# alexisvannson/GraphNet_Classifier

Hardware: AMD Instinct MI355X
Metric: edges aggregated/sec (GraphNet forward) (higher is better)
Workload: dtype f32; 1 GPU; c3: 1M nodes / 10M edges (6250 graphs x 160 nodes x 1600 edges), D=64, 2 GN blocks; graphs=6250, nodes=1000000, edges=10000000, n_blocks=2, width=64, step=CSR build + GraphNet.forward, inputs resident in HBM

## Files before the change

### graphnet_classifier_amd/GNN.py

```python
from __future__ import annotations

import os

import torch
import torch.nn as nn
from torch import Tensor

from . import functional as Fn
from . import native
from .MLP import MLP, default_device, require_gpu_param
from .topology import GraphTopology, get_destination_csr, get_topology


WSPLIT = os.environ.get("GNC_NO_WSPLIT") is None
READOUT_HIP = os.environ.get("GNC_NO_READOUT_KERNEL") is None
FUSED_AGG = os.environ.get("GNC_NO_FUSED_AGG") is None


def scatter_sum(src: Tensor, index: Tensor, dim: int = 0, dim_size: int | None = None) -> Tensor:
    if dim != 0:
        raise NotImplementedError("fallback scatter_sum currently supports dim=0 only")
    if src.ndim == 1:
        src = src.unsqueeze(-1)
    if dim_size is None:
        dim_size = int(index.max().item()) + 1 if index.numel() > 0 else 0
    dev = src.device if src.is_cuda else default_device()
    if dev.type != "cuda":
        raise RuntimeError("scatter_sum: no GPU visible and no CPU fallback exists")
    out_device = src.device
    csr = get_destination_csr(index, dim_size, dev)
    src = src.to(device=dev, dtype=torch.float32)
# ... 11 lines not shown

class EdgeProcessor(nn.Module):
    def __init__(self, in_dim_node: int, in_dim_edge: int, hidden_dim: int = 128, hidden_layers: int = 2,
                 activation: str = "ReLU", initializer: None | str = None, norm_type: None | str = "LayerNorm"):
        super().__init__()
        self.edge_processor = MLP(2 * in_dim_node + in_dim_edge, in_dim_edge, hidden_dim, hidden_layers, activation,
                                  initializer, norm_type)

    def forward(self, src, dest, edge_attr, u=None, batch=None):
        dev = require_gpu_param(self.edge_processor.model[0].weight, "EdgeProcessor")
        back = edge_attr.device
        src, dest, edge_attr = (t.to(device=dev, dtype=torch.float32) for t in (src, dest, edge_attr))
        out = self.edge_processor.forward_segments([(src, None), (dest, None), (edge_attr, None)], residual=edge_attr)
        return out if back == dev else out.to(back)

    def forward_sorted(self, x: Tensor, topo: GraphTopology, edge_attr: Tensor, aggregate: bool = False):
        mlp = self.edge_processor
        norm = mlp.model[-1] if mlp.norm_type is not None else None
        lin = mlp._linears()
        trainable_split = mlp.activation_name == "ReLU" or not torch.is_grad_enabled()
        if (WSPLIT and trainable_split and not isinstance(norm, nn.BatchNorm1d) and mlp.activation_name in native.ACTIVATIONS
                and lin[0].in_features == 2 * x.size(1) + edge_attr.size(1) and x.size(1) % 4 == 0):
            ln = (norm.weight, norm.bias, norm.eps) if isinstance(norm, nn.LayerNorm) else None
            if aggregate and not torch.is_grad_enabled():
                return Fn.edge_processor_wsplit_aggregated(x, edge_attr, topo, [m.weight for m in lin], [m.bias for m in lin],
                                                           ln, mlp.activation_name, mlp._act_param())
            if aggregate:
                return Fn.edge_processor_wsplit(x, edge_attr, topo, [m.weight for m in lin], [m.bias for m in lin], ln,
                                                mlp.activation_name, mlp._act_param(), with_agg=True)
            return Fn.edge_processor_wsplit(x, edge_attr, topo, [m.weight for m in lin],
                                            [m.bias for m in lin], ln, mlp.activation_name, mlp._act_param())
        out = mlp.forward_segments(
            [(x, topo.src_sorted), (x, topo.dst_sorted), (edge_attr, None)], residual=edge_attr, rows=topo.num_edges)
        return (out, None) if aggregate else out


class NodeProcessor(nn.Module):
    def __init__(self, in_dim_node: int, in_dim_edge: int, hidden_dim: int = 128, hidden_layers: int = 2,
                 activation: str = "ReLU", initializer: None | str = None, norm_type: None | str = "LayerNorm"):
        super().__init__()
        self.node_processor = MLP(in_dim_node + in_dim_edge, in_dim_node, hidden_dim, hidden_layers, activation,
# ... 26 lines not shown

    def forward(self, x: Tensor, edge_index: Tensor, edge_attr: Tensor | None = None, u=None, batch=None):
        dev = require_gpu_param(next(self.parameters()), "MetaLayer")
        back = x.device
        x = x.to(device=dev, dtype=torch.float32)
        edge_attr = edge_attr.to(device=dev, dtype=torch.float32)
        topo = get_topology(edge_index, x.size(0), dev)
        e_sorted = Fn.permute_rows(edge_attr, topo.perm, topo.inv_perm)
        x, e_sorted = self.forward_sorted(x, topo, e_sorted)
        edge_attr = Fn.permute_rows(e_sorted, topo.inv_perm, topo.perm)
        x, edge_attr = _poison_if_deferred(topo, x), _poison_if_deferred(topo, edge_attr)
        if back != dev:
            x, edge_attr = x.to(back), edge_attr.to(back)
        return x, edge_attr, u

    def forward_sorted(self, x: Tensor, topo: GraphTopology, edge_attr: Tensor):
        agg = None
        if self.edge_model is not None:
            if (FUSED_AGG and self.node_model is not None
                    and isinstance(self.edge_model, EdgeProcessor) and isinstance(self.node_model, NodeProcessor)):
                edge_attr, agg = self.edge_model.forward_sorted(x, topo, edge_attr, aggregate=True)
            else:
                edge_attr = self.edge_model.forward_sorted(x, topo, edge_attr)
        if self.node_model is not None:
            if agg is not None:
                x = self.node_model.forward_sorted(x, topo, edge_attr, agg)
            else:
                x = self.node_model.forward_sorted(x, topo, edge_attr)
        return x, edge_attr


def build_GN_block(in_dim_node: int, in_dim_edge: int, hidden_dim_node: int = 128, hidden_dim_edge: int = 128,
                   hidden_layers_node: int = 2, hidden_layers_edge: int = 2, activation: str = "ReLU",
                   initializer: None | str = None, norm_type: None | str = "LayerNorm"):
    return MetaLayer(
        edge_model=EdgeProcessor(in_dim_node, in_dim_edge, hidden_dim_edge, hidden_layers_edge, activation,
# ... 17 lines not shown
    def forward(self, x, edge_index, edge_attr):
        if len(self.blocks) == 0:
            return x, edge_attr
        dev = require_gpu_param(next(self.parameters()), "GraphProcessor")
        back = x.device
        x = x.to(device=dev, dtype=torch.float32)
        edge_attr = edge_attr.to(device=dev, dtype=torch.float32)
        topo = get_topology(edge_index, x.size(0), dev)
        x, e_sorted = self.forward_sorted(x, topo, Fn.permute_rows(edge_attr, topo.perm, topo.inv_perm))
        edge_attr = Fn.permute_rows(e_sorted, topo.inv_perm, topo.perm)
        x, edge_attr = _poison_if_deferred(topo, x), _poison_if_deferred(topo, edge_attr)
        if back != dev:
            x, edge_attr = x.to(back), edge_attr.to(back)
        return x, edge_attr

    def forward_sorted(self, x, topo: GraphTopology, edge_attr):
        for block in self.blocks:
            x, edge_attr = block.forward_sorted(x, topo, edge_attr)
        return x, edge_attr


class GraphNet(nn.Module):
    def __init__(self, **kwargs):
        super().__init__()
        num_global_features = kwargs.get("num_global_features", 0)
        num_local_features = kwargs.get("num_local_features", 3)
        space_dim = kwargs.get("space_dim", 2)
        in_dim_node = num_local_features + num_global_features
        in_dim_edge = 1 + space_dim
        out_dim = kwargs.get("out_channels", 1)
        n_blocks = kwargs.get("n_blocks", 10)
        out_dim_node = kwargs.get("out_dim_node", 128)
        out_dim_edge = kwargs.get("out_dim_edge", 128)
# ... 19 lines not shown
                                initializer=initializer, norm_type=norm_type)
        self.edge_encoder = MLP(in_dim_edge, out_dim_edge, hidden_dim_edge, hidden_layers_edge, activation=activation,
                                initializer=initializer, norm_type=norm_type)
        self.graph_processor = GraphProcessor(n_blocks, out_dim_node, out_dim_edge, hidden_dim_processor_node,
                                              hidden_dim_processor_edge, hidden_layers_processor_node,
                                              hidden_layers_processor_edge, activation=activation,
                                              initializer=initializer, norm_type=norm_type)
        self.node_decoder = MLP(out_dim_node, out_dim, hidden_dim_decoder, hidden_layers_decoder, norm_type=None)

    def forward_device(self, x: Tensor, pos: Tensor, topo: GraphTopology) -> Tensor:
        out = self.node_encoder.forward_segments([(x.view(x.size(0), -1), None)])
        edge_attr = self.edge_encoder.forward_edge_features(pos, topo.src_sorted, topo.dst_sorted)
        if edge_attr is None:
            edge_attr = Fn.edge_features(pos, topo.src_sorted, topo.dst_sorted)
            edge_attr = self.edge_encoder.forward_segments([(edge_attr, None)])
        out, _ = self.graph_processor.forward_sorted(out, topo, edge_attr)
        out = self.node_decoder.forward_segments([(out, None)])
        return _poison_if_deferred(topo, out)

    def forward(self, x, pos, edge_index):
        dev = require_gpu_param(self.node_encoder.model[0].weight, "GraphNet")
        back = x.device
        x = x.to(device=dev, dtype=torch.float32)
        pos = pos.to(device=dev, dtype=torch.float32)
        topo = get_topology(edge_index, x.size(0), dev)
        out = self.forward_device(x, pos, topo)
        return out if back == dev else out.to(back)


class CapturedForward:

# ... 142 lines not shown
```

### graphnet_classifier_amd/csrc/mlp_device.h

```cpp
#pragma once
#include "gnc_common.h"

namespace gnc_mlp {

typedef float f32x16 __attribute__((ext_vector_type(16)));
typedef float f32x4 __attribute__((ext_vector_type(4)));

constexpr int KC = 64;
constexpr int LDSW = 68;
constexpr int RPW = 32;

__device__ __forceinline__ f32x16 mfma(float a, float b, f32x16 c) {
  return __builtin_amdgcn_mfma_f32_32x32x2f32(a, b, c, 0, 0, 0);
}

__device__ __forceinline__ void wave_lds_fence() {
  asm volatile("s_waitcnt lgkmcnt(0)" ::: "memory");
}

__device__ __forceinline__ float activate(float x, int act, float p) {
  switch (act) {
    case GNC_ACT_RELU: return x < 0.f ? 0.f : x;
    case GNC_ACT_IDENTITY: return x;
    case GNC_ACT_TANH: return tanhf(x);
// ... 745 lines not shown
  float* g_sum;
  int ld_g_sum;
};

__host__ __device__ inline int ldw_of(const gnc_mlp_desc_t& d, int l) { return d.ld_weight[l] ? d.ld_weight[l] : d.in_dim[l]; }

inline int tiles_for(int width) {
  const int t = (width + 31) / 32;
  return t <= 1 ? 1 : t <= 2 ? 2 : t <= 4 ? 4 : 8;
}

int validate_desc(const gnc_mlp_desc_t* d, bool check_ptrs);
int launch_resident_dual(const float* x, int64_t ld_x, int64_t rows, const float* wa, int64_t ld_wa, const float* wb, int64_t ld_wb,
                         int in_dim, int out_dim, float* out_a, float* out_b, int64_t ld_out, hipStream_t stream, bool* launched);
int launch_resident(const gnc_mlp_desc_t& d, int T, bool narrow_out, hipStream_t stream, bool* launched,
                    bool probe_only = false);
int launch_stream(const gnc_mlp_desc_t& d, int T, bool narrow_out, hipStream_t stream, bool* launched,
                  bool probe_only = false);
int launch_stream16(const gnc_mlp_desc_t& d, hipStream_t stream, bool* launched, bool probe_only = false);
int launch_col16(const gnc_mlp_desc_t& d, hipStream_t stream, bool* launched, bool probe_only = false);
int64_t col16_max_rows();
int64_t bwd_col16_max_rows();
bool bwd_col16_supported(const gnc_mlp_desc_t& d);
int bwd_col16_ln_partial_rows(int64_t rows);
int launch_bwd_col16(const gnc_mlp_bwd_desc_t& bd, hipStream_t stream);
bool bwd_col16_persist_supported(const gnc_mlp_desc_t& d);
int bwd_col16_persist_ln_partial_rows(int64_t rows);
int launch_bwd_col16_persist(const gnc_mlp_bwd_desc_t& bd, hipStream_t stream);
bool bwd_stream16_supported(const gnc_mlp_desc_t& d, bool want_dx);
int bwd_stream16_ln_partial_rows(int64_t rows);
int launch_bwd_stream16(const gnc_mlp_desc_t& d, const BwdArgs& b, hipStream_t stream, bool saved = false);
// ... 3 lines not shown
```

### graphnet_classifier_amd/csrc/mlp_fused.hip

```cpp
#include <stdlib.h>

#include "mlp_device.h"

using namespace gnc_mlp;

namespace {

constexpr int WAVES = 4;
constexpr int NT = WAVES * 64;
constexpr int RPB = RPW * WAVES;

__device__ __forceinline__ void stage_rows(float* abuf, const gnc_mlp_segment_t& seg, int64_t row0, int64_t rows,
                                           int c0, int ncol4, bool vec_ok, int lane) {
  const int c4 = lane & 15;
  const int rs = lane >> 4;
  if (c4 < ncol4) {
#pragma unroll
    for (int p = 0; p < RPW / 4; ++p) {
      const int j = p * 4 + rs;
      const int64_t r = row0 + j;
      f32x4 v = {0.f, 0.f, 0.f, 0.f};
      if (r < rows) {
        const int64_t tr = seg.index ? (int64_t)seg.index[r] : r;
        if (!seg.index || (uint64_t)tr < (uint64_t)seg.table_rows)
// ... 232 lines not shown
    rc = launch_stream(probe, T, narrow_out, nullptr, &ok, true);
    if (rc) return rc;
  }
  if (!ok && T == 8) {
    rc = launch_stream16(probe, nullptr, &ok, true);
    if (rc) return rc;
  }
  if (!ok) {
    gnc::set_error("gnc_mlp_agg_supported: needs the weights-resident W-split shape (1 MATMUL + 2 ADD segments, residual = "
                   "the MATMUL segment, widths 33..64) or a 65..128-wide description of the streaming kernel");
    return GNC_ERR_UNSUPPORTED;
  }
  return GNC_OK;
}

namespace {
bool small16(const gnc_mlp_desc_t& d, int T) {
  static const bool off = getenv("GNC_NO_SMALL16") != nullptr;
  return !off && T == 4 && d.rows <= (int64_t)2 * 16 * gnc::num_cu();
}
}

extern "C" int gnc_mlp_save_act_supported(const gnc_mlp_desc_t* desc) {
  int rc = validate_desc(desc, false);
  if (rc) return rc;
  const int L = desc->num_linear;
  int T = tiles_for(desc->out_dim[0]);
  const int od = desc->out_dim[L - 1];
  const bool narrow_out = od <= 32;
  if (!narrow_out && tiles_for(od) > T) T = tiles_for(od);
// ... 167 lines not shown
```

### graphnet_classifier_amd/csrc/mlp_resident.hip

```cpp
#include <stdlib.h>

#include "mlp_device.h"

using namespace gnc_mlp;

#ifdef GNC_PHASE_PROBE
__device__ unsigned long long gnc_phase_probe[4096 * 12];
extern "C" int gnc_phase_probe_read(void* dst, size_t bytes) {
  return (int)hipMemcpyFromSymbol(dst, HIP_SYMBOL(gnc_phase_probe), bytes);
}
#define PROBE_BEGIN() unsigned long long pr_acc[8] = {0, 0, 0, 0, 0, 0, 0, 0}, pr_tp, pr_tn; \
  const unsigned long long pr_c0 = __builtin_readcyclecounter(), pr_w0 = wall_clock64()
#define PROBE_TILE() pr_tp = __builtin_readcyclecounter()
#define PROBE(k) do { pr_tn = __builtin_readcyclecounter(); pr_acc[k] += pr_tn - pr_tp; pr_tp = pr_tn; } while (0)
#define PROBE_END() do { if ((threadIdx.x & 63) == 0) {                                                      \
    unsigned long long* o = gnc_phase_probe + (blockIdx.x * (blockDim.x >> 6) + (threadIdx.x >> 6)) * 12;    \
    for (int k = 0; k < 8; ++k) o[k] = pr_acc[k];                                                            \
    o[8] = __builtin_readcyclecounter() - pr_c0; o[9] = wall_clock64() - pr_w0; } } while (0)
#else
#define PROBE_BEGIN() do {} while (0)
#define PROBE_TILE() do {} while (0)
#define PROBE(k) do {} while (0)
#define PROBE_END() do {} while (0)
#endif

namespace {

constexpr int RWAVES = 8;
constexpr int RNT = RWAVES * 64;

template <int HT, int OT, int NMM, int NADD, bool RESREG, bool AGG = false, bool SAVE = false, bool FULL = false, int EF = 0, bool DUAL = false,
          int SPLIT = 0>
__global__ __launch_bounds__(RNT) void mlp_resident_kernel(const gnc_mlp_desc_t d, const int num_wtiles,
                                                           const int total_chunks) {
  extern __shared__ __attribute__((aligned(16))) float lds[];
  constexpr int WT = HT > OT ? HT : OT;
  constexpr int CH = WT * 32 * LDSW;
  static_assert(SPLIT == 0 || (WT == 2 && NMM == 1 && !DUAL && (SPLIT == 1 || NADD == 0)), "split shapes");
  constexpr int nf32 = SPLIT == 1 ? 0 : NMM;
  __bf16* const wsp = reinterpret_cast<__bf16*>(lds + nf32 * CH);
  auto wsplit = [&](int chunk) -> const __bf16* { return wsp + (chunk - nf32) * 3 * SPLANE; };
  constexpr int PSTRIDE = WT * 32;
  constexpr int NS = NMM + NADD;
  const int tid = threadIdx.x;
  const int lane = tid & 63;
  const int wave = __builtin_amdgcn_readfirstlane(tid >> 6);
  const int i = lane & 31;
// ... 156 lines not shown
  const int col_out = c4 * 4;
  const bool vec_out = FULL || ((out_dim % 4 == 0) && (d.ld_out % 4 == 0) && ((reinterpret_cast<uintptr_t>(d.out) & 15u) == 0));
  const uint32_t out_lane_off = (uint32_t)(rs * d.ld_out + col_out) * 4u;
  const uint32_t res_lane_off = (uint32_t)(rs * d.ld_residual + (col_out < d.ld_residual ? col_out : 0)) * 4u;

  auto agg_ids = [&](int t) -> int {
    int r = t * RPW + (lane & 31);
    r = r < rows ? r : rows - 1;
    return d.agg_index[r];
  };
  int aid = 0, aid_next = 0;
  float agg_acc = 0.f;
  int agg_cur = -1, agg_first_dst = -1;
  bool agg_first = true;
  if constexpr (AGG) aid = agg_ids(wt < last_wt ? wt : last_wt);

  PROBE_BEGIN();
  while (wt < wt_end) {
    PROBE_TILE();
    const int row0 = wt * RPW;
    const int nwt = wt + stride;
    if constexpr (AGG) aid_next = agg_ids(nwt < last_wt ? nwt : last_wt);

    f32x16 hid[HT];
    f32x16 res[RESREG ? HT : 1];
    init_bias<HT>(hid, pbuf, h);
#pragma unroll
    for (int s = 0; s < NMM; ++s) {
      bool interleaved = false;
      if constexpr (EF == 1) ef_stage();
// ... 140 lines not shown
      if constexpr (RESREG) {
#pragma unroll
        for (int t = 0; t < OT && t < HT; ++t) o[t] += res[t < HT ? t : 0];
      }
      compiler_lds_barrier();
      tiles_to_lds<OT>(o, abuf, i, h);
      PROBE(5);
    }
    compiler_lds_barrier();
    if constexpr (AGG) {
      const int valid = rows - row0 < RPW ? rows - row0 : RPW;
      int prv = __shfl_up(aid, 1, 64);
      prv = lane == 0 ? agg_cur : prv;
      const unsigned long long vmask = valid >= 32 ? 0xffffffffull : ((1ull << valid) - 1ull);
      const unsigned long long bnd = __ballot(aid != prv) & vmask;
      float rowv[RPW];
#pragma unroll
      for (int r = 0; r < RPW; ++r) rowv[r] = abuf[r * LDSW + lane];
      auto agg_row = [&](int r) {
        if ((bnd >> r) & 1ull) {
          if (agg_cur >= 0) {
            if (agg_first) {
              agg_first = false;
              agg_first_dst = agg_cur;
            } else if (lane < out_dim) {
              float* dstp = d.agg_out + (int64_t)agg_cur * d.ld_agg;
              asm volatile("s_nop 4\n\tglobal_store_dword %0, %1, %2\n\ts_nop 0" ::"v"(lane * 4), "v"(agg_acc), "s"(dstp) : "memory");
            }
          }
          agg_cur = __builtin_amdgcn_readlane(aid, r);
// ... 17 lines not shown
      aid = aid_next;
    }
    if constexpr (EF == 1) {
      asm volatile("" ::"v"(ef_ps), "v"(ef_pd), "v"(ef_s), "v"(ef_d));
    } else if constexpr (EF == 2) {
      asm volatile("" ::"v"(n3_row.x), "v"(n3_row.y), "v"(n3_row.z));
    } else {
#pragma unroll
      for (int p = 0; p < NP; ++p) asm volatile("" ::"v"(cur[p]));
    }
#pragma unroll
    for (int s = 1; s < NS; ++s) asm volatile("" ::"v"(offs[s]));
    asm volatile("" ::"v"(off0));
    if constexpr (AGG) asm volatile("" ::"v"(aid_next));

    {
      f32x4 outv[NP];
#pragma unroll
      for (int p = 0; p < NP; ++p) outv[p] = *reinterpret_cast<const f32x4*>(abuf + (p * 4 + rs) * LDSW + col_out);
      if (!RESREG && d.residual) {
        f32x4 rv[NP];
        load_tile_rows(rv, d.residual, d.ld_residual, row0, rows, res_lane_off);
#pragma unroll
        for (int p = 0; p < NP; ++p) outv[p] += rv[p];
      }
      if (vec_out) {
        if (col_out < out_dim) {
          if (row0 + RPW <= rows) {
            uint32_t r0b;
            const __amdgpu_buffer_rsrc_t ow = full_tile_window(d.out, row0, rows, d.ld_out, &r0b);
#pragma unroll
// ... 33 lines not shown
    }
    compiler_lds_barrier();
    PROBE(6);
    wt = nwt;
  }
  if constexpr (AGG) {
    if (lane == 0) {
      d.agg_fix[2 * gwave] = agg_first ? agg_cur : agg_first_dst;
      d.agg_fix[2 * gwave + 1] = agg_cur;
    }
  }
  PROBE_END();
}

template <int HT, int OT, int NMM, int NADD, bool RESREG, bool AGG = false, bool SAVE = false, bool FULL = false, int EF = 0, bool DUAL = false,
          int SPLIT = 0>
int launch(const gnc_mlp_desc_t& d, int total_chunks, size_t smem, hipStream_t stream) {
  void (*const kernel)(const gnc_mlp_desc_t, const int, const int) = &mlp_resident_kernel<HT, OT, NMM, NADD, RESREG, AGG, SAVE, FULL, EF, DUAL, SPLIT>;
  static bool attr_set = false;
  if (!attr_set) {
    int rc = gnc::check_hip(hipFuncSetAttribute(reinterpret_cast<const void*>(kernel), hipFuncAttributeMaxDynamicSharedMemorySize, 160 * 1024),
                            "hipFuncSetAttribute(MaxDynamicSharedMemorySize)");
    if (rc) return rc;
    attr_set = true;
  }
  const int64_t num_wtiles = gnc::ceil_div(d.rows, RPW);
  int64_t grid = gnc::ceil_div(num_wtiles, RWAVES);
  if (grid > gnc::num_cu()) grid = gnc::num_cu();
  if constexpr (AGG) grid = gnc::num_cu();
  kernel<<<dim3((unsigned)grid), dim3(RNT), smem, stream>>>(d, (int)num_wtiles, total_chunks);
  return gnc::check_launch("mlp_resident_kernel");
}

template <int HT, int OT, int NMM, int NADD, bool RESREG, bool AGG = false, bool SAVE = false, bool FULL = false, int EF = 0>
int launch_cls(int split, const gnc_mlp_desc_t& d, int total_chunks, size_t smem, hipStream_t stream) {
  if constexpr (HT == 2 && OT == 2 && NMM == 1 && NADD == 2 && RESREG) {
    if (split == 1) return launch<HT, OT, NMM, NADD, RESREG, AGG, SAVE, FULL, EF, false, 1>(d, total_chunks, smem, stream);
  }
  if constexpr (HT == 2 && OT == 2 && NMM == 1 && NADD == 0 && !RESREG && !AGG && !FULL) {
    if (split == 2) return launch<HT, OT, NMM, NADD, RESREG, AGG, SAVE, FULL, EF, false, 2>(d, total_chunks, smem, stream);
  }
  if (split) return GNC_ERR_UNSUPPORTED;
  return launch<HT, OT, NMM, NADD, RESREG, AGG, SAVE, FULL, EF>(d, total_chunks, smem, stream);
}

bool al16(const void* p) { return (reinterpret_cast<uintptr_t>(p) & 15u) == 0; }

}

extern "C" int gnc_mlp_agg_fix_len(void) { return 2 * gnc::num_cu() * RWAVES; }

int gnc_mlp::launch_resident_dual(const float* x, int64_t ld_x, int64_t rows, const float* wa, int64_t ld_wa, const float* wb,
                                  int64_t ld_wb, int in_dim, int out_dim, float* out_a, float* out_b, int64_t ld_out,
                                  hipStream_t stream, bool* launched) {
  *launched = false;
  static const bool disabled = getenv("GNC_MLP_NO_RESIDENT") != nullptr;
  if (disabled || rows < 1 || rows >= INT32_MAX || in_dim < 1 || in_dim > KC || out_dim <= 32 || out_dim > KC || out_dim % 4 != 0 ||
      ld_x % 4 != 0 || ld_x < in_dim || ld_out % 4 != 0 || ld_out < out_dim || ld_wa < in_dim || ld_wb < in_dim || ld_wa > INT32_MAX ||
// ... 13 lines not shown
  d.ld_weight[1] = (int32_t)ld_wb;
  d.in_dim[0] = in_dim;
  d.out_dim[0] = out_dim;
  d.in_dim[1] = in_dim;
  d.out = out_a;
  d.save_act[0] = out_b;
  d.ld_out = (int32_t)ld_out;
  d.rows = rows;
  const int total_chunks = 2;
  const size_t floats = (size_t)total_chunks * 2 * 32 * LDSW + (size_t)(1 + 2) * 2 * 32 + (size_t)RWAVES * RPW * LDSW;
  *launched = true;
  return launch<2, 2, 1, 0, false, false, false, false, 0, true>(d, total_chunks, floats * sizeof(float), stream);
}

int gnc_mlp::launch_resident(const gnc_mlp_desc_t& d, int T, bool narrow_out, hipStream_t stream, bool* launched,
                             bool probe_only) {
  *launched = false;
  static const bool disabled = getenv("GNC_MLP_NO_RESIDENT") != nullptr;
  if (disabled) return GNC_OK;
  if (T > 2 || d.rows >= INT32_MAX) return GNC_OK;
  const int L = d.num_linear;
  const int od = d.out_dim[L - 1];
  if (L > 1 && d.activation != GNC_ACT_RELU) return GNC_OK;
  int nmm = 0, nadd = 0;
  bool n3 = false;
  for (int s = 0; s < d.num_segments; ++s) {
    const gnc_mlp_segment_t& g = d.seg[s];
    if (d.ef_pos && s == 0) continue;
    if (s == 0 && d.num_segments == 1 && !g.index && g.mode == GNC_SEG_MATMUL && g.width == 3 && g.ld == 3 &&
        (reinterpret_cast<uintptr_t>(g.ptr) & 3u) == 0 && d.rows * 12 <= 0xffffffffll && !d.residual && !d.save_act[0] && !d.agg_out &&
        !narrow_out && L >= 2 && T == 2) {
      n3 = true;
// ... 66 lines not shown
    if (d.agg_out && !(nadd == 2 && resreg && d.agg_index && d.agg_fix && d.ld_agg >= od)) return GNC_OK;
    if (nadd == 2 && !resreg) return GNC_OK;
    *launched = true;
    if (probe_only) return GNC_OK;
    if (nmm == 2)
      return resreg ? launch<2, 2, 2, 0, true, false, true>(d, total_chunks, smem, stream)
                    : launch<2, 2, 2, 0, false, false, true>(d, total_chunks, smem, stream);
    if (d.agg_out) return full64 ? launch_cls<2, 2, 1, 2, true, true, true, true>(split, d, total_chunks, smem, stream)
                                 : launch_cls<2, 2, 1, 2, true, true, true>(split, d, total_chunks, smem, stream);
    if (nadd == 2) return launch_cls<2, 2, 1, 2, true, false, true>(split, d, total_chunks, smem, stream);
    return resreg ? launch<2, 2, 1, 0, true, false, true>(d, total_chunks, smem, stream)
                  : launch_cls<2, 2, 1, 0, false, false, true>(split, d, total_chunks, smem, stream);
  }
  if (d.agg_out) {
    if (!(nadd == 2 && nmm == 1 && resreg && !narrow_out && d.agg_index && d.agg_fix && d.ld_agg >= od)) return GNC_OK;
    *launched = true;
    if (probe_only) return GNC_OK;
    if (T == 2 && full64) return launch_cls<2, 2, 1, 2, true, true, false, true>(split, d, total_chunks, smem, stream);
    return T == 2 ? launch_cls<2, 2, 1, 2, true, true>(split, d, total_chunks, smem, stream)
                  : launch<1, 1, 1, 2, true, true>(d, total_chunks, smem, stream);
  }
  if (probe_only) {
    *launched = true;
    return GNC_OK;
  }
#define GNC_RES(HT_, NMM_, NADD_)                                                             \
  do {                                                                                        \
    *launched = true;                                                                         \
    return resreg ? launch<HT_, HT_, NMM_, NADD_, true>(d, total_chunks, smem, stream)        \
                  : launch<HT_, HT_, NMM_, NADD_, false>(d, total_chunks, smem, stream);      \
  } while (0)
  if (narrow_out) {
// ... 20 lines not shown
```

### graphnet_classifier_amd/functional.py

```python
from __future__ import annotations

import torch
import torch.nn.functional as F

import os

from . import native

HIP_BACKWARD = os.environ.get("GNC_TORCH_BACKWARD") is None


def _node_projections(x, w0, dn):
    return native.dual_projection(x, w0[:, :dn], w0[:, dn:2 * dn])


class _ScatterSumCSR(torch.autograd.Function):
    @staticmethod
    def forward(ctx, src, rowptr, perm, dst_of_row, num_nodes):
        ctx.save_for_backward(dst_of_row)
        return native.scatter_sum_csr(src, rowptr, perm, num_nodes)

    @staticmethod
    def backward(ctx, grad_out):
        (dst_of_row,) = ctx.saved_tensors
# ... 385 lines not shown
            dbeta, dgamma = sums[0][:od], sums[0][od:]
        else:
            dbeta, dgamma = r["ln_sums"] if r["ln_sums"] is not None else native.colsum_pair(grad_out, r["yhat"])
        grads[2 + 2 * num_linear] = dgamma
        grads[2 + 2 * num_linear + 1] = dbeta
    return tuple(g if n else None for g, n in zip(grads, need))


def edge_processor_wsplit(x, e, topo, weights, biases, ln, activation="ReLU", act_param=0.0, with_agg=False):
    meta = (topo.src_sorted, topo.dst_sorted, len(weights), activation, float(act_param),
            float(ln[2]) if ln is not None else 0.0, ln is not None, bool(with_agg), torch.is_grad_enabled())
    args = list(weights) + list(biases) + ([ln[0], ln[1]] if ln is not None else [])
    return _EdgeProcessorWSplit.apply(meta, topo, x, e, *args)


def edge_processor_wsplit_aggregated(x, e, topo, weights, biases, ln, activation="ReLU", act_param=0.0):
    dn = x.size(1)
    w0 = weights[0]
    ps, pd = _node_projections(x, w0, dn)
    return native.mlp_forward([(ps, topo.src_sorted), (pd, topo.dst_sorted), (e, None)], [w0[:, 2 * dn:]] + list(weights[1:]),
                              list(biases), ln=ln, activation=activation, act_param=act_param, residual=e, rows=e.size(0),
                              modes=[native.SEG_ADD, native.SEG_ADD, native.SEG_MATMUL],
                              aggregate=(topo.dst_sorted, topo.rowptr, topo.num_nodes))


class _Readout(torch.autograd.Function):

    @staticmethod
    def forward(ctx, y, w1, b1, w2, b2, w3, b3):
        logits, h1, h2 = native.readout_forward(y, w1, b1, w2, b2, w3, b3)
        ctx.save_for_backward(y, w1, w2, w3, h1, h2)
        ctx.has_bias = (b1 is not None, b2 is not None, b3 is not None)
        return logits

    @staticmethod
    def backward(ctx, grad_logits):
        y, w1, w2, w3, h1, h2 = ctx.saved_tensors
        need = ctx.needs_input_grad
# ... 16 lines not shown
```

### graphnet_classifier_amd/native.py

```python
from __future__ import annotations

import ctypes
import os
from ctypes import POINTER, Structure, c_char_p, c_double, c_float, c_int32, c_int64, c_size_t, c_void_p

import torch

LIB_NAME = "libgnc_hip.so"
LIB_PATH = os.path.join(os.path.dirname(os.path.abspath(__file__)), LIB_NAME)

GNC_MAX_SEGMENTS = 4
GNC_MAX_LINEAR = 8
ABI_VERSION = 20

ACTIVATIONS = {
    "ReLU": 0, "Identity": 1, "Tanh": 2, "Sigmoid": 3, "SiLU": 4, "GELU": 5, "LeakyReLU": 6, "ELU": 7,
}

_SIGNATURES = {
    "gnc_abi_version": (c_int32, []),
    "gnc_last_error_string": (c_char_p, []),
    "gnc_target_arch": (c_char_p, []),
    "gnc_mlp_agg_supported": (c_int32, [c_void_p]),
    "gnc_mlp_edge_features_supported": (c_int32, [c_void_p]),
    "gnc_mlp_operands_in_place_supported": (c_int32, [c_void_p]),
    "gnc_mlp_save_act_supported": (c_int32, [c_void_p]),
    "gnc_mlp_agg_fix_len": (c_int32, []),
    "gnc_mlp_small_batch_supported": (c_int32, [c_void_p]),
    "gnc_mlp_small_batch_max_rows": (c_int64, []),
    "gnc_mlp_projection_t2_f32": (c_int32, [c_void_p, c_int64, c_void_p, c_int64, c_int64, c_void_p, c_int64, c_int32, c_int32, c_void_p,
                                            c_int64, c_void_p]),
    "gnc_mlp_dual_projection_f32": (c_int32, [c_void_p, c_int64, c_int64, c_void_p, c_int64, c_void_p, c_int64, c_int32, c_int32,
                                              c_void_p, c_void_p, c_int64, c_void_p]),
    "gnc_mlp_backward_small_batch_supported": (c_int32, [c_void_p]),
    "gnc_readout_forward_f32": (c_int32, [c_void_p, c_int64, c_void_p, c_int64, c_void_p, c_int32, c_void_p, c_int64, c_void_p, c_int32,
                                          c_void_p, c_int64, c_void_p, c_int32, c_void_p, c_void_p, c_void_p, c_void_p, c_void_p]),
    "gnc_readout_backward_f32": (c_int32, [c_void_p, c_void_p, c_int64, c_void_p, c_int64, c_int32, c_void_p, c_int64, c_int32, c_void_p,
                                           c_int64, c_int32, c_void_p, c_void_p, c_void_p, c_void_p, c_void_p, c_void_p, c_void_p, c_void_p,
# ... 446 lines not shown

def _backward_reads_saved_act(lib, desc, any_tensor, need_dx: bool = True) -> bool:
    bd = MlpBwdDesc()
    ctypes.memmove(ctypes.byref(bd.fwd), ctypes.byref(desc), ctypes.sizeof(MlpDesc))
    ptr = any_tensor.data_ptr()
    for l in range(desc.num_linear - 1):
        bd.act[l] = ptr
    bd.act_given, bd.dx = 1, (ptr if need_dx else None)
    if lib.gnc_mlp_backward_fused_rows(ctypes.byref(bd.fwd)) > 0:
        bd.dw_partial[0] = ptr
    return lib.gnc_mlp_backward_saved_act_honoured(ctypes.byref(bd)) == 1


def mlp_forward(segments, weights, biases, ln=None, activation: str = "ReLU", act_param: float = 0.0,
                residual: torch.Tensor | None = None, rows: int | None = None, modes=None, aggregate=None,
                save_act: list | None = None, save_need_dx: bool = True):
    lib = load_library()
    given = (segments, weights, biases, residual, rows, modes)
    small = _rows_of(segments, rows) <= _small_batch_rows(lib)
    raw = not small and save_act is None and aggregate is None
    segs, weights, biases, residual, rows, modes = _prepare_mlp(*given, vector_rows=not (small or raw))
    dev = segs[0][0].device
    out = torch.empty(rows, weights[-1].size(0), dtype=torch.float32, device=dev)
    desc = make_mlp_desc(segs, weights, biases, ln, activation, act_param, residual, out, rows)
    if raw and any(t.data_ptr() % 16 or _ld(t) % 4 for t in [sg[0] for sg in segs] + weights) and \
            lib.gnc_mlp_operands_in_place_supported(ctypes.byref(desc)) != 0:
        segs, weights, biases, residual, rows, modes = _prepare_mlp(*given)
        desc = make_mlp_desc(segs, weights, biases, ln, activation, act_param, residual, out, rows)
    if small and lib.gnc_mlp_small_batch_supported(ctypes.byref(desc)) != 0:
        segs, weights, biases, residual, rows, modes = _prepare_mlp(*given)
        desc = make_mlp_desc(segs, weights, biases, ln, activation, act_param, residual, out, rows)
    if (save_act is not None and SAVE_ACT and rows > 0 and len(weights) >= 2
            and lib.gnc_mlp_save_act_supported(ctypes.byref(desc)) == 0 and _backward_reads_saved_act(lib, desc, out, save_need_dx)):
        for l in range(len(weights) - 1):
            a = torch.empty(rows, weights[l].size(0), dtype=torch.float32, device=dev)
            desc.save_act[l] = a.data_ptr()
            save_act.append(a)
    agg = fix = None
    if aggregate is not None:
        dst_of_row, rowptr, num_nodes = aggregate
        _require_cuda(dst_of_row, rowptr)
        if rows > 0 and lib.gnc_mlp_agg_supported(ctypes.byref(desc)) == 0:
            agg = torch.empty(num_nodes, out.size(1), dtype=torch.float32, device=dev)
            fix = torch.empty(lib.gnc_mlp_agg_fix_len(), dtype=torch.int32, device=dev)
            desc.agg_out, desc.ld_agg = agg.data_ptr(), _ld(agg)
            desc.agg_index, desc.agg_fix = dst_of_row.contiguous().data_ptr(), fix.data_ptr()
    flops = 2.0 * rows * sum(w.size(0) * w.size(1) for w in weights)
    with torch.cuda.device(dev):
        nadd = sum(1 for m in modes if m == SEG_ADD)
        _check(_launch(f"mlp_fused_in{weights[0].size(1)}{'+%dadd' % nadd if nadd else ''}_h{weights[0].size(0)}"
                       f"_out{weights[-1].size(0)}_L{len(weights)}", out,
                       lambda: lib.gnc_mlp_forward_f32(ctypes.byref(desc), _stream(out)), flops),
               "gnc_mlp_forward_f32")
        if agg is not None:
            _check(lib.gnc_agg_fixup_f32(out.data_ptr(), _ld(out), rowptr.data_ptr(), fix.data_ptr(), fix.numel(), num_nodes,
                                         out.size(1), agg.data_ptr(), _ld(agg), _stream(out)), "gnc_agg_fixup_f32")
    return (out, agg) if aggregate is not None else out


FOLD_EDGE_FEATURES = os.environ.get("GNC_NO_K6_FOLD") is None


def mlp_forward_edge_features(pos: torch.Tensor, src: torch.Tensor, dst: torch.Tensor, weights, biases, ln=None,
                              activation: str = "ReLU", act_param: float = 0.0):
    lib = load_library()
    if not FOLD_EDGE_FEATURES or pos.dim() != 2 or pos.size(1) != 2 or src.numel() == 0:
        return None
    _require_cuda(pos, src, dst)
    if src.dtype != torch.int32 or dst.dtype != torch.int32:
        raise TypeError("edge endpoint ids must be int32")
    pos = pos.float().contiguous()
    src, dst = src.contiguous(), dst.contiguous()
# ... 420 lines not shown
```

### include/gnc_hip.h

```cpp
#ifndef GNC_HIP_H
#define GNC_HIP_H

#include <stddef.h>
#include <stdint.h>

#ifdef __cplusplus
extern "C" {
#endif

#define GNC_ABI_VERSION 20

enum {
  GNC_OK = 0,
  GNC_ERR_INVALID_ARGUMENT = -1,
  GNC_ERR_UNSUPPORTED = -2,
  GNC_ERR_WORKSPACE = -3,
  GNC_ERR_HIP = -4
};

#define GNC_MAX_SEGMENTS 4
#define GNC_MAX_LINEAR 8

enum { GNC_ACT_RELU = 0, GNC_ACT_IDENTITY = 1, GNC_ACT_TANH = 2, GNC_ACT_SIGMOID = 3,
       GNC_ACT_SILU = 4, GNC_ACT_GELU = 5, GNC_ACT_LEAKY_RELU = 6, GNC_ACT_ELU = 7 };
// ... 67 lines not shown
  const int32_t* agg_index;
  int32_t* agg_fix;
  float* save_act[GNC_MAX_LINEAR];
  const float* ef_pos;
  const int32_t* ef_src;
  const int32_t* ef_dst;
  int64_t ef_nodes;
  int32_t ef_space_dim;
} gnc_mlp_desc_t;

size_t gnc_sizeof_mlp_desc(void);
int gnc_mlp_supported(const gnc_mlp_desc_t* desc );
int gnc_mlp_forward_f32(const gnc_mlp_desc_t* desc , void* stream);
int gnc_mlp_agg_supported(const gnc_mlp_desc_t* desc );
int gnc_mlp_agg_fix_len(void);
int gnc_mlp_operands_in_place_supported(const gnc_mlp_desc_t* desc );
int gnc_mlp_edge_features_supported(const gnc_mlp_desc_t* desc );
int gnc_mlp_small_batch_supported(const gnc_mlp_desc_t* desc );
int gnc_mlp_projection_t2_f32(const float* a, int64_t ld_a, const float* b, int64_t ld_b, int64_t rows, const float* w, int64_t ld_w,
                              int32_t hidden, int32_t dn, float* out, int64_t ld_out, void* stream);
int64_t gnc_mlp_small_batch_max_rows(void);
int gnc_mlp_dual_projection_f32(const float* x, int64_t ld_x, int64_t rows, const float* wa, int64_t ld_wa, const float* wb,
                                int64_t ld_wb, int32_t in_dim, int32_t out_dim, float* out_a, float* out_b, int64_t ld_out,
                                void* stream);
int gnc_mlp_save_act_supported(const gnc_mlp_desc_t* desc );
int gnc_agg_fixup_f32(const float* src, int64_t ld_src, const int32_t* rowptr, const int32_t* fix, int32_t n_fix,
                      int64_t num_nodes, int32_t feat_dim, float* out, int64_t ld_out, void* stream);

typedef struct gnc_mlp_bwd_desc {
  gnc_mlp_desc_t fwd;
// ... 97 lines not shown
```

Measured before the change: 2.977 billion edges/s.

## Skip dead edge-feature store in last GN block, keep only aggregate boundary rows

The last GraphNet block's updated edge features are never consumed after node aggregation, so a new aggregate-only variant of the resident fused MLP kernel is added. It skips writing the per-edge output to HBM and stores only the rows at the first and last destination of each work tile, which the aggregation fixup pass still reads. This removes one 10M×64 f32 write in the final block, at the cost of another kernel instantiation and a ballot per chunk.

```diff
diff --git a/graphnet_classifier_amd/GNN.py b/graphnet_classifier_amd/GNN.py
--- a/graphnet_classifier_amd/GNN.py
+++ b/graphnet_classifier_amd/GNN.py
@@ -15,6 +15,7 @@
 WSPLIT = os.environ.get("GNC_NO_WSPLIT") is None
 READOUT_HIP = os.environ.get("GNC_NO_READOUT_KERNEL") is None
 FUSED_AGG = os.environ.get("GNC_NO_FUSED_AGG") is None
+DROP_DEAD_EDGE_STORE = os.environ.get("GNC_NO_DEAD_EDGE_STORE") is None
 
 
 def scatter_sum(src: Tensor, index: Tensor, dim: int = 0, dim_size: int | None = None) -> Tensor:
@@ -56,7 +57,8 @@
         out = self.edge_processor.forward_segments([(src, None), (dest, None), (edge_attr, None)], residual=edge_attr)
         return out if back == dev else out.to(back)
 
-    def forward_sorted(self, x: Tensor, topo: GraphTopology, edge_attr: Tensor, aggregate: bool = False):
+    def forward_sorted(self, x: Tensor, topo: GraphTopology, edge_attr: Tensor, aggregate: bool = False,
+                       need_edges: bool = True):
         mlp = self.edge_processor
         norm = mlp.model[-1] if mlp.norm_type is not None else None
         lin = mlp._linears()
@@ -66,7 +68,7 @@
             ln = (norm.weight, norm.bias, norm.eps) if isinstance(norm, nn.LayerNorm) else None
             if aggregate and not torch.is_grad_enabled():
                 return Fn.edge_processor_wsplit_aggregated(x, edge_attr, topo, [m.weight for m in lin], [m.bias for m in lin],
-                                                           ln, mlp.activation_name, mlp._act_param())
+                                                           ln, mlp.activation_name, mlp._act_param(), store_edges=need_edges)
             if aggregate:
                 return Fn.edge_processor_wsplit(x, edge_attr, topo, [m.weight for m in lin], [m.bias for m in lin], ln,
                                                 mlp.activation_name, mlp._act_param(), with_agg=True)
@@ -123,12 +125,12 @@
             x, edge_attr = x.to(back), edge_attr.to(back)
         return x, edge_attr, u
 
-    def forward_sorted(self, x: Tensor, topo: GraphTopology, edge_attr: Tensor):
+    def forward_sorted(self, x: Tensor, topo: GraphTopology, edge_attr: Tensor, need_edges: bool = True):
         agg = None
         if self.edge_model is not None:
             if (FUSED_AGG and self.node_model is not None
                     and isinstance(self.edge_model, EdgeProcessor) and isinstance(self.node_model, NodeProcessor)):
-                edge_attr, agg = self.edge_model.forward_sorted(x, topo, edge_attr, aggregate=True)
+                edge_attr, agg = self.edge_model.forward_sorted(x, topo, edge_attr, aggregate=True, need_edges=need_edges)
             else:
                 edge_attr = self.edge_model.forward_sorted(x, topo, edge_attr)
         if self.node_model is not None:
@@ -176,9 +178,10 @@
             x, edge_attr = x.to(back), edge_attr.to(back)
         return x, edge_attr
 
-    def forward_sorted(self, x, topo: GraphTopology, edge_attr):
-        for block in self.blocks:
-            x, edge_attr = block.forward_sorted(x, topo, edge_attr)
+    def forward_sorted(self, x, topo: GraphTopology, edge_attr, need_edges: bool = True):
+        last = len(self.blocks) - 1
+        for k, block in enumerate(self.blocks):
+            x, edge_attr = block.forward_sorted(x, topo, edge_attr, need_edges=need_edges or k < last)
         return x, edge_attr
 
 
@@ -228,7 +231,7 @@
         if edge_attr is None:
             edge_attr = Fn.edge_features(pos, topo.src_sorted, topo.dst_sorted)
             edge_attr = self.edge_encoder.forward_segments([(edge_attr, None)])
-        out, _ = self.graph_processor.forward_sorted(out, topo, edge_attr)
+        out, _ = self.graph_processor.forward_sorted(out, topo, edge_attr, need_edges=not DROP_DEAD_EDGE_STORE)
         out = self.node_decoder.forward_segments([(out, None)])
         return _poison_if_deferred(topo, out)
 
diff --git a/graphnet_classifier_amd/csrc/mlp_device.h b/graphnet_classifier_amd/csrc/mlp_device.h
--- a/graphnet_classifier_amd/csrc/mlp_device.h
+++ b/graphnet_classifier_amd/csrc/mlp_device.h
@@ -783,7 +783,7 @@
 int launch_resident_dual(const float* x, int64_t ld_x, int64_t rows, const float* wa, int64_t ld_wa, const float* wb, int64_t ld_wb,
                          int in_dim, int out_dim, float* out_a, float* out_b, int64_t ld_out, hipStream_t stream, bool* launched);
 int launch_resident(const gnc_mlp_desc_t& d, int T, bool narrow_out, hipStream_t stream, bool* launched,
-                    bool probe_only = false);
+                    bool probe_only = false, bool agg_only = false);
 int launch_stream(const gnc_mlp_desc_t& d, int T, bool narrow_out, hipStream_t stream, bool* launched,
                   bool probe_only = false);
 int launch_stream16(const gnc_mlp_desc_t& d, hipStream_t stream, bool* launched, bool probe_only = false);
diff --git a/graphnet_classifier_amd/csrc/mlp_fused.hip b/graphnet_classifier_amd/csrc/mlp_fused.hip
--- a/graphnet_classifier_amd/csrc/mlp_fused.hip
+++ b/graphnet_classifier_amd/csrc/mlp_fused.hip
@@ -270,6 +270,56 @@
   return GNC_OK;
 }
 
+extern "C" int gnc_mlp_agg_only_supported(const gnc_mlp_desc_t* desc) {
+  int rc = gnc_mlp_agg_supported(desc);
+  if (rc) return rc;
+  const int L = desc->num_linear;
+  int T = tiles_for(desc->out_dim[0]);
+  const int od = desc->out_dim[L - 1];
+  const bool narrow_out = od <= 32;
+  if (!narrow_out && tiles_for(od) > T) T = tiles_for(od);
+  gnc_mlp_desc_t probe = *desc;
+  int32_t dummy_i = 0;
+  float dummy_f = 0.f;
+  if (!probe.agg_out) probe.agg_out = &dummy_f;
+  if (!probe.agg_index) probe.agg_index = &dummy_i;
+  if (!probe.agg_fix) probe.agg_fix = &dummy_i;
+  if (probe.ld_agg < od) probe.ld_agg = od;
+  bool ok = false;
+  rc = launch_resident(probe, T, narrow_out, nullptr, &ok, true, true);
+  if (rc) return rc;
+  if (!ok) {
+    gnc::set_error("gnc_mlp_agg_only_supported: needs the 64-wide W-split edge processor (1 MATMUL + 2 ADD segments, residual = "
+                   "the MATMUL segment, three Linear layers, LayerNorm) without save_act");
+    return GNC_ERR_UNSUPPORTED;
+  }
+  return GNC_OK;
+}
+
+extern "C" int gnc_mlp_forward_agg_only_f32(const gnc_mlp_desc_t* desc, void* stream) {
+  int rc = validate_desc(desc, true);
+  if (rc) return rc;
+  if (!desc->agg_out || !desc->agg_index || !desc->agg_fix) {
+    gnc::set_error("gnc_mlp_forward_agg_only_f32: agg_out, agg_index and agg_fix are required");
+    return GNC_ERR_INVALID_ARGUMENT;
+  }
+  rc = gnc_mlp_agg_only_supported(desc);
+  if (rc) return rc;
+  if (desc->rows == 0) return GNC_OK;
+  const int L = desc->num_linear;
+  int T = tiles_for(desc->out_dim[0]);
+  const int od = desc->out_dim[L - 1];
+  const bool narrow_out = od <= 32;
+  if (!narrow_out && tiles_for(od) > T) T = tiles_for(od);
+  bool launched = false;
+  rc = launch_resident(*desc, T, narrow_out, (hipStream_t)stream, &launched, false, true);
+  if (!rc && !launched) {
+    gnc::set_error("gnc_mlp_forward_agg_only_f32: the weights-resident kernel did not take the launch");
+    rc = GNC_ERR_UNSUPPORTED;
+  }
+  return rc;
+}
+
 namespace {
 bool small16(const gnc_mlp_desc_t& d, int T) {
   static const bool off = getenv("GNC_NO_SMALL16") != nullptr;
diff --git a/graphnet_classifier_amd/csrc/mlp_resident.hip b/graphnet_classifier_amd/csrc/mlp_resident.hip
--- a/graphnet_classifier_amd/csrc/mlp_resident.hip
+++ b/graphnet_classifier_amd/csrc/mlp_resident.hip
@@ -30,7 +30,7 @@
 constexpr int RNT = RWAVES * 64;
 
 template <int HT, int OT, int NMM, int NADD, bool RESREG, bool AGG = false, bool SAVE = false, bool FULL = false, int EF = 0, bool DUAL = false,
-          int SPLIT = 0>
+          int SPLIT = 0, bool AGGONLY = false>
 __global__ __launch_bounds__(RNT) void mlp_resident_kernel(const gnc_mlp_desc_t d, const int num_wtiles,
                                                            const int total_chunks) {
   extern __shared__ __attribute__((aligned(16))) float lds[];
@@ -217,6 +217,16 @@
   int agg_cur = -1, agg_first_dst = -1;
   bool agg_first = true;
   if constexpr (AGG) aid = agg_ids(wt < last_wt ? wt : last_wt);
+  static_assert(!AGGONLY || (AGG && FULL && !SAVE && !DUAL), "aggregate-only: the FULL AGG inference instance");
+  int keep_lo = -1, keep_hi = -1;
+  if constexpr (AGGONLY) {
+    if (wt < wt_end) {
+      const int last_row = wt_end * RPW < rows ? wt_end * RPW - 1 : rows - 1;
+      keep_lo = d.agg_index[wt * RPW];
+      keep_hi = d.agg_index[last_row];
+    }
+  }
+  uint32_t keep_rows = 0;
 
   PROBE_BEGIN();
   while (wt < wt_end) {
@@ -387,6 +397,7 @@
       prv = lane == 0 ? agg_cur : prv;
       const unsigned long long vmask = valid >= 32 ? 0xffffffffull : ((1ull << valid) - 1ull);
       const unsigned long long bnd = __ballot(aid != prv) & vmask;
+      if constexpr (AGGONLY) keep_rows = (uint32_t)(__ballot(aid == keep_lo || aid == keep_hi) & vmask);
       float rowv[RPW];
 #pragma unroll
       for (int r = 0; r < RPW; ++r) rowv[r] = abuf[r * LDSW + lane];
@@ -434,7 +445,15 @@
     asm volatile("" ::"v"(off0));
     if constexpr (AGG) asm volatile("" ::"v"(aid_next));
 
-    {
+    if constexpr (AGGONLY) {
+      if (keep_rows) {
+#pragma unroll
+        for (int p = 0; p < NP; ++p) {
+          const f32x4 v = *reinterpret_cast<const f32x4*>(abuf + (p * 4 + rs) * LDSW + col_out);
+          if ((keep_rows >> (p * 4 + rs)) & 1u) hidden_window_store<true>(v, out_lane_off, row_window(d.out, row0 + 4 * p, rows, d.ld_out));
+        }
+      }
+    } else {
       f32x4 outv[NP];
 #pragma unroll
       for (int p = 0; p < NP; ++p) outv[p] = *reinterpret_cast<const f32x4*>(abuf + (p * 4 + rs) * LDSW + col_out);
@@ -498,9 +517,9 @@
 }
 
 template <int HT, int OT, int NMM, int NADD, bool RESREG, bool AGG = false, bool SAVE = false, bool FULL = false, int EF = 0, bool DUAL = false,
-          int SPLIT = 0>
+          int SPLIT = 0, bool AGGONLY = false>
 int launch(const gnc_mlp_desc_t& d, int total_chunks, size_t smem, hipStream_t stream) {
-  void (*const kernel)(const gnc_mlp_desc_t, const int, const int) = &mlp_resident_kernel<HT, OT, NMM, NADD, RESREG, AGG, SAVE, FULL, EF, DUAL, SPLIT>;
+  void (*const kernel)(const gnc_mlp_desc_t, const int, const int) = &mlp_resident_kernel<HT, OT, NMM, NADD, RESREG, AGG, SAVE, FULL, EF, DUAL, SPLIT, AGGONLY>;
   static bool attr_set = false;
   if (!attr_set) {
     int rc = gnc::check_hip(hipFuncSetAttribute(reinterpret_cast<const void*>(kernel), hipFuncAttributeMaxDynamicSharedMemorySize, 160 * 1024),
@@ -516,16 +535,17 @@
   return gnc::check_launch("mlp_resident_kernel");
 }
 
-template <int HT, int OT, int NMM, int NADD, bool RESREG, bool AGG = false, bool SAVE = false, bool FULL = false, int EF = 0>
+template <int HT, int OT, int NMM, int NADD, bool RESREG, bool AGG = false, bool SAVE = false, bool FULL = false, int EF = 0,
+          bool AGGONLY = false>
 int launch_cls(int split, const gnc_mlp_desc_t& d, int total_chunks, size_t smem, hipStream_t stream) {
   if constexpr (HT == 2 && OT == 2 && NMM == 1 && NADD == 2 && RESREG) {
-    if (split == 1) return launch<HT, OT, NMM, NADD, RESREG, AGG, SAVE, FULL, EF, false, 1>(d, total_chunks, smem, stream);
+    if (split == 1) return launch<HT, OT, NMM, NADD, RESREG, AGG, SAVE, FULL, EF, false, 1, AGGONLY>(d, total_chunks, smem, stream);
   }
   if constexpr (HT == 2 && OT == 2 && NMM == 1 && NADD == 0 && !RESREG && !AGG && !FULL) {
     if (split == 2) return launch<HT, OT, NMM, NADD, RESREG, AGG, SAVE, FULL, EF, false, 2>(d, total_chunks, smem, stream);
   }
   if (split) return GNC_ERR_UNSUPPORTED;
-  return launch<HT, OT, NMM, NADD, RESREG, AGG, SAVE, FULL, EF>(d, total_chunks, smem, stream);
+  return launch<HT, OT, NMM, NADD, RESREG, AGG, SAVE, FULL, EF, false, 0, AGGONLY>(d, total_chunks, smem, stream);
 }
 
 bool al16(const void* p) { return (reinterpret_cast<uintptr_t>(p) & 15u) == 0; }
@@ -569,8 +589,9 @@
 }
 
 int gnc_mlp::launch_resident(const gnc_mlp_desc_t& d, int T, bool narrow_out, hipStream_t stream, bool* launched,
-                             bool probe_only) {
+                             bool probe_only, bool agg_only) {
   *launched = false;
+  if (agg_only && (!d.agg_out || d.save_act[0])) return GNC_OK;
   static const bool disabled = getenv("GNC_MLP_NO_RESIDENT") != nullptr;
   if (disabled) return GNC_OK;
   if (T > 2 || d.rows >= INT32_MAX) return GNC_OK;
@@ -667,8 +688,10 @@
   }
   if (d.agg_out) {
     if (!(nadd == 2 && nmm == 1 && resreg && !narrow_out && d.agg_index && d.agg_fix && d.ld_agg >= od)) return GNC_OK;
+    if (agg_only && !(T == 2 && full64)) return GNC_OK;
     *launched = true;
     if (probe_only) return GNC_OK;
+    if (agg_only) return launch_cls<2, 2, 1, 2, true, true, false, true, 0, true>(split, d, total_chunks, smem, stream);
     if (T == 2 && full64) return launch_cls<2, 2, 1, 2, true, true, false, true>(split, d, total_chunks, smem, stream);
     return T == 2 ? launch_cls<2, 2, 1, 2, true, true>(split, d, total_chunks, smem, stream)
                   : launch<1, 1, 1, 2, true, true>(d, total_chunks, smem, stream);
diff --git a/graphnet_classifier_amd/functional.py b/graphnet_classifier_amd/functional.py
--- a/graphnet_classifier_amd/functional.py
+++ b/graphnet_classifier_amd/functional.py
@@ -423,14 +423,14 @@
     return _EdgeProcessorWSplit.apply(meta, topo, x, e, *args)
 
 
-def edge_processor_wsplit_aggregated(x, e, topo, weights, biases, ln, activation="ReLU", act_param=0.0):
+def edge_processor_wsplit_aggregated(x, e, topo, weights, biases, ln, activation="ReLU", act_param=0.0, store_edges=True):
     dn = x.size(1)
     w0 = weights[0]
     ps, pd = _node_projections(x, w0, dn)
     return native.mlp_forward([(ps, topo.src_sorted), (pd, topo.dst_sorted), (e, None)], [w0[:, 2 * dn:]] + list(weights[1:]),
                               list(biases), ln=ln, activation=activation, act_param=act_param, residual=e, rows=e.size(0),
                               modes=[native.SEG_ADD, native.SEG_ADD, native.SEG_MATMUL],
-                              aggregate=(topo.dst_sorted, topo.rowptr, topo.num_nodes))
+                              aggregate=(topo.dst_sorted, topo.rowptr, topo.num_nodes), agg_only=not store_edges)
 
 
 class _Readout(torch.autograd.Function):
diff --git a/graphnet_classifier_amd/native.py b/graphnet_classifier_amd/native.py
--- a/graphnet_classifier_amd/native.py
+++ b/graphnet_classifier_amd/native.py
@@ -22,6 +22,8 @@
     "gnc_last_error_string": (c_char_p, []),
     "gnc_target_arch": (c_char_p, []),
     "gnc_mlp_agg_supported": (c_int32, [c_void_p]),
+    "gnc_mlp_agg_only_supported": (c_int32, [c_void_p]),
+    "gnc_mlp_forward_agg_only_f32": (c_int32, [c_void_p, c_void_p]),
     "gnc_mlp_edge_features_supported": (c_int32, [c_void_p]),
     "gnc_mlp_operands_in_place_supported": (c_int32, [c_void_p]),
     "gnc_mlp_save_act_supported": (c_int32, [c_void_p]),
@@ -498,7 +500,7 @@
 
 def mlp_forward(segments, weights, biases, ln=None, activation: str = "ReLU", act_param: float = 0.0,
                 residual: torch.Tensor | None = None, rows: int | None = None, modes=None, aggregate=None,
-                save_act: list | None = None, save_need_dx: bool = True):
+                save_act: list | None = None, save_need_dx: bool = True, agg_only: bool = False):
     lib = load_library()
     given = (segments, weights, biases, residual, rows, modes)
     small = _rows_of(segments, rows) <= _small_batch_rows(lib)
@@ -529,17 +531,19 @@
             fix = torch.empty(lib.gnc_mlp_agg_fix_len(), dtype=torch.int32, device=dev)
             desc.agg_out, desc.ld_agg = agg.data_ptr(), _ld(agg)
             desc.agg_index, desc.agg_fix = dst_of_row.contiguous().data_ptr(), fix.data_ptr()
+    agg_only = agg_only and agg is not None and lib.gnc_mlp_agg_only_supported(ctypes.byref(desc)) == 0
+    forward = lib.gnc_mlp_forward_agg_only_f32 if agg_only else lib.gnc_mlp_forward_f32
     flops = 2.0 * rows * sum(w.size(0) * w.size(1) for w in weights)
     with torch.cuda.device(dev):
         nadd = sum(1 for m in modes if m == SEG_ADD)
         _check(_launch(f"mlp_fused_in{weights[0].size(1)}{'+%dadd' % nadd if nadd else ''}_h{weights[0].size(0)}"
                        f"_out{weights[-1].size(0)}_L{len(weights)}", out,
-                       lambda: lib.gnc_mlp_forward_f32(ctypes.byref(desc), _stream(out)), flops),
-               "gnc_mlp_forward_f32")
+                       lambda: forward(ctypes.byref(desc), _stream(out)), flops),
+               forward.__name__)
         if agg is not None:
             _check(lib.gnc_agg_fixup_f32(out.data_ptr(), _ld(out), rowptr.data_ptr(), fix.data_ptr(), fix.numel(), num_nodes,
                                          out.size(1), agg.data_ptr(), _ld(agg), _stream(out)), "gnc_agg_fixup_f32")
-    return (out, agg) if aggregate is not None else out
+    return (None if agg_only else out, agg) if aggregate is not None else out
 
 
 FOLD_EDGE_FEATURES = os.environ.get("GNC_NO_K6_FOLD") is None
diff --git a/include/gnc_hip.h b/include/gnc_hip.h
--- a/include/gnc_hip.h
+++ b/include/gnc_hip.h
@@ -105,6 +105,8 @@
 int gnc_mlp_forward_f32(const gnc_mlp_desc_t* desc , void* stream);
 int gnc_mlp_agg_supported(const gnc_mlp_desc_t* desc );
 int gnc_mlp_agg_fix_len(void);
+int gnc_mlp_agg_only_supported(const gnc_mlp_desc_t* desc );
+int gnc_mlp_forward_agg_only_f32(const gnc_mlp_desc_t* desc , void* stream);
 int gnc_mlp_operands_in_place_supported(const gnc_mlp_desc_t* desc );
 int gnc_mlp_edge_features_supported(const gnc_mlp_desc_t* desc );
 int gnc_mlp_small_batch_supported(const gnc_mlp_desc_t* desc );
```

Result: faster. 3.044 billion edges/s (median of 6 runs) (+2.2%).
